# erincatto/solver2d

Hardware: NVIDIA B200
Metric: constraint_iters_per_sec (higher is better)
Workload: dtype f32

## Files before the change

### include/s2b_device.h

```cpp
#pragma once

#include <stddef.h>
#include <stdint.h>

#ifdef __cplusplus
extern "C"
{
#endif

typedef struct s2bWorld s2bWorld;

#if defined(__GNUC__)
	#define S2B_API __attribute__((visibility("default")))
#else
	#define S2B_API
#endif


#define S2B_ROW_VALID 0x1
#define S2B_BODY_ADD_FORCE 0x8

typedef struct s2bBodyRow
{
	int32_t index;
// ... 110 lines not shown
	int32_t constraintCount;
	int32_t jointCount;
	int32_t groupCount;
	int32_t overflowCount;
	int32_t treeHeight;
	int32_t movedCount;
	int32_t pairPassCount;
	int32_t kernelLaunches;
	int32_t graphReplays;
	int32_t graphCaptures;
	int64_t scratchBytes;
	int32_t regionCount;
	int32_t cutCount;
	int32_t cutGroupCount;
	int32_t recolouredCount;
} s2bCounters;


S2B_API s2bWorld* s2b_world_create(int cudaDevice, int solverType);
S2B_API void s2b_world_destroy(s2bWorld* world);

S2B_API void s2b_set_gravity(s2bWorld* world, float gx, float gy);
S2B_API void s2b_set_schedule(s2bWorld* world, int schedule);
S2B_API void s2b_set_max_colors(s2bWorld* world, int maxColors);
S2B_API void s2b_set_persistent(s2bWorld* world, int enable);
S2B_API void s2b_set_warm_gather(s2bWorld* world, int enable);
S2B_API void s2b_set_graph(s2bWorld* world, int enable);
S2B_API void s2b_set_regions(s2bWorld* world, int mode);
S2B_API void s2b_set_dataflow(s2bWorld* world, int enable);

// ... 65 lines not shown
```

### solver2d_b200/csrc/device/broadphase.cu

```cuda
#include "s2b_internal.cuh"

#include <cub/cub.cuh>
#include <thrust/iterator/counting_iterator.h>

#include <algorithm>

struct BroadScratch
{
	DevArray<int> validFlag;
	DevArray<int> leafShape;
	DevArray<unsigned> mortonIn, mortonOut;
	DevArray<int> leafIn, leafOut;
	DevArray<int> counters;
	DevArray<int> boundsBits;
	DevArray<int2> children;
	DevArray<int> parent;
	DevArray<float4> nodeBox;
	DevArray<float4> pairBox;
	DevArray<int> visit;
	DevArray<int> nodeHeight;
	DevArray<int> movedLeaves;
	DevArray<int> movedFlag;
	DevArray<int> largeShapes;
	DevArray<unsigned long long> newKey;
	DevArray<int2> newShapes;
	DevArray<int> keepFlag, keepSlots;
	DevArray<unsigned long long> mergeKeyIn, mergeKeyOut;
	DevArray<int> mergeSrcIn, mergeSrcOut;
	DevArray<char> cubTemp;
	int newPairCap = 0;
	bool treeValid = false;
	int treeShapeCap = 0;
	int treeReuses = 0;
	DevArray<unsigned long long> pairHash;
	unsigned long long hashMask = 0;
	unsigned long long hashVersion = ~0ull;
// ... 19 lines not shown
}

void s2bFreeBroadScratch(s2bWorld* w)
{
	BroadScratch* b = w->broad;
	if (b == nullptr)
	{
		return;
	}
	b->validFlag.release();
	b->leafShape.release();
	b->mortonIn.release();
	b->mortonOut.release();
	b->leafIn.release();
	b->leafOut.release();
	b->counters.release();
	b->boundsBits.release();
	b->children.release();
	b->parent.release();
	b->nodeBox.release();
	b->visit.release();
	b->nodeHeight.release();
	b->movedLeaves.release();
	b->movedFlag.release();
	b->newKey.release();
	b->newShapes.release();
	b->keepFlag.release();
	b->keepSlots.release();
	b->mergeKeyIn.release();
	b->mergeKeyOut.release();
	b->mergeSrcIn.release();
	b->mergeSrcOut.release();
	b->cubTemp.release();
	b->pairBox.release();
	b->largeShapes.release();
	b->pairHash.release();
	for (int i = 0; i < 2; ++i)
	{
		if (b->evSearch[i] != nullptr)
		{
			cudaEventDestroy(b->evSearch[i]);
		}
	}
	if (b->searchDone != nullptr)
	{
		cudaEventDestroy(b->searchDone);
	}
	delete b;
	w->broad = nullptr;
}

enum
{
	BC_LEAVES = 0,
	BC_NEW_PAIRS = 1,
	BC_KEPT = 2,
	BC_MOVED = 3,
	BC_HEIGHT = 4,
	BC_LARGE = 5,
	BC_SIZE = 8
};


__device__ __forceinline__ int s2bFloatToOrdered(float f)
{
	int i = __float_as_int(f);
	return i >= 0 ? i : i ^ 0x7FFFFFFF;
}

__device__ __forceinline__ float s2bOrderedToFloat(int i)
{
	return __int_as_float(i >= 0 ? i : i ^ 0x7FFFFFFF);
}

// ... 123 lines not shown
}

__device__ __forceinline__ int s2bPairKind(int t1, int t2)
{
	const int CAP = S2B_SHAPE_CAPSULE, CIR = S2B_SHAPE_CIRCLE, POL = S2B_SHAPE_POLYGON, SEG = S2B_SHAPE_SEGMENT;
	if (t1 == SEG && t2 == SEG)
	{
		return 0;
	}
	bool primary = (t1 == CIR && t2 == CIR) || (t1 == CAP && t2 == CIR) || (t1 == CAP && t2 == CAP) || (t1 == POL && t2 == CIR) ||
				   (t1 == POL && t2 == CAP) || (t1 == POL && t2 == POL) || (t1 == SEG && t2 != SEG);
	return primary ? 1 : 2;
}


__global__ void s2bFlagValidShapes(ShapeView s, int* validFlag)
{
	int i = blockIdx.x * blockDim.x + threadIdx.x;
	if (i < s.capacity)
	{
		validFlag[i] = (s.head[i].x & S2B_ROW_VALID) ? 1 : 0;
	}
}

__global__ void s2bSceneBounds(ShapeView s, const int* leafShape, const int* counters, int* boundsBits)
{
	int n = counters[BC_LEAVES];
	int k = blockIdx.x * blockDim.x + threadIdx.x;
	float minx = 3.0e38f, miny = 3.0e38f, maxx = -3.0e38f, maxy = -3.0e38f;
	if (k < n)
	{
		float4 f = s.fat[leafShape[k]];
		float cx = 0.5f * (f.x + f.z), cy = 0.5f * (f.y + f.w);
		minx = maxx = cx;
		miny = maxy = cy;
	}
	for (int o = 16; o > 0; o >>= 1)
	{
		minx = fminf(minx, __shfl_xor_sync(0xFFFFFFFFu, minx, o));
		miny = fminf(miny, __shfl_xor_sync(0xFFFFFFFFu, miny, o));
		maxx = fmaxf(maxx, __shfl_xor_sync(0xFFFFFFFFu, maxx, o));
		maxy = fmaxf(maxy, __shfl_xor_sync(0xFFFFFFFFu, maxy, o));
	}
	if ((threadIdx.x & 31) == 0)
	{
		atomicMin(boundsBits + 0, s2bFloatToOrdered(minx));
		atomicMin(boundsBits + 1, s2bFloatToOrdered(miny));
		atomicMax(boundsBits + 2, s2bFloatToOrdered(maxx));
		atomicMax(boundsBits + 3, s2bFloatToOrdered(maxy));
	}
}

__global__ void s2bMortonCodes(ShapeView s, const int* leafShape, const int* counters, const int* boundsBits, unsigned* morton,
							   int* leafIndex, int capacity)
{
	int n = counters[BC_LEAVES];
	int k = blockIdx.x * blockDim.x + threadIdx.x;
	if (k >= capacity)
	{
		return;
	}
	if (k >= n)
	{
		morton[k] = 0xFFFFFFFFu;
		leafIndex[k] = k;
		return;
	}
	float minx = s2bOrderedToFloat(boundsBits[0]), miny = s2bOrderedToFloat(boundsBits[1]);
	float maxx = s2bOrderedToFloat(boundsBits[2]), maxy = s2bOrderedToFloat(boundsBits[3]);
	float4 f = s.fat[leafShape[k]];
	float cx = 0.5f * (f.x + f.z), cy = 0.5f * (f.y + f.w);
	float ex = fmaxf(maxx - minx, 1.0e-6f), ey = fmaxf(maxy - miny, 1.0e-6f);
	float ux = fminf(fmaxf((cx - minx) / ex, 0.0f), 1.0f);
	float uy = fminf(fmaxf((cy - miny) / ey, 0.0f), 1.0f);
	unsigned qx = (unsigned)(ux * 32767.0f), qy = (unsigned)(uy * 32767.0f);
	morton[k] = (s2bExpandBits(qx) | (s2bExpandBits(qy) << 1)) & 0x7FFFFFFFu;
	leafIndex[k] = k;
}

__device__ __forceinline__ int s2bDelta(const unsigned* codes, int n, int i, int j)
{
	if (j < 0 || j >= n)
	{
		return -1;
	}
	unsigned a = codes[i], b = codes[j];
	if (a == b)
	{
		return 32 + __clz((unsigned)i ^ (unsigned)j);
	}
	return __clz(a ^ b);
}

__global__ void s2bBuildRadixTree(const unsigned* codes, const int* counters, int2* children, int* parent)
{
	int n = counters[BC_LEAVES];
	int i = blockIdx.x * blockDim.x + threadIdx.x;
	if (i >= n - 1)
	{
		return;
	}
	int d = (s2bDelta(codes, n, i, i + 1) - s2bDelta(codes, n, i, i - 1)) >= 0 ? 1 : -1;
	int deltaMin = s2bDelta(codes, n, i, i - d);
	int lmax = 2;
	while (s2bDelta(codes, n, i, i + lmax * d) > deltaMin)
	{
		lmax <<= 1;
	}
	int l = 0;
	for (int t = lmax >> 1; t >= 1; t >>= 1)
	{
		if (s2bDelta(codes, n, i, i + (l + t) * d) > deltaMin)
		{
			l += t;
		}
	}
	int j = i + l * d;
	int deltaNode = s2bDelta(codes, n, i, j);
	int s = 0;
	int t = l;
	do
	{
		t = (t + 1) >> 1;
		if (s2bDelta(codes, n, i, i + (s + t) * d) > deltaNode)
		{
			s += t;
		}
	} while (t > 1);
	int gamma = i + s * d + min(d, 0);
	int left = min(i, j) == gamma ? (n - 1) + gamma : gamma;
	int right = max(i, j) == gamma + 1 ? (n - 1) + gamma + 1 : gamma + 1;
	children[i] = make_int2(left, right);
	parent[left] = i;
	parent[right] = i;
	if (i == 0)
	{
		parent[0] = -1;
	}
}

__global__ void s2bRefit(ShapeView s, const int* leafShape, const int* sortedLeaf, const int* counters, const int2* children,
						 const int* parent, float4* nodeBox, float4* pairBox, int* visit, int* nodeHeight, int* countersOut)
{
	int n = counters[BC_LEAVES];
	int k = blockIdx.x * blockDim.x + threadIdx.x;
	if (k >= n)
	{
		return;
	}
	int node = (n - 1) + k;
	float4 box = s.fat[leafShape[sortedLeaf[k]]];
	nodeBox[node] = box;
	nodeHeight[node] = 0;
	if (n == 1)
	{
		countersOut[BC_HEIGHT] = 0;
		return;
	}
	int p = parent[node];
	while (p >= 0)
	{
		__threadfence();
		int arrived = atomicAdd(visit + p, 1);
		if (arrived == 0)
		{
			return;
		}
		int2 ch = children[p];
		float4 a = __ldcg(nodeBox + ch.x), b = __ldcg(nodeBox + ch.y);
		box = make_float4(fminf(a.x, b.x), fminf(a.y, b.y), fmaxf(a.z, b.z), fmaxf(a.w, b.w));
		nodeBox[p] = box;
		pairBox[2 * p] = a;
		pairBox[2 * p + 1] = b;
		int h = 1 + max(__ldcg(nodeHeight + ch.x), __ldcg(nodeHeight + ch.y));
		nodeHeight[p] = h;
		if (p == 0)
		{
			countersOut[BC_HEIGHT] = h;
		}
		p = parent[p];
	}
}


__device__ __forceinline__ void s2bBlockAppend(bool take, int value, int* list, int* count)
{
	__shared__ int warpOffset[32];
	__shared__ int blockBase;
	unsigned takers = __ballot_sync(0xFFFFFFFFu, take);
	int lane = threadIdx.x & 31, warp = threadIdx.x >> 5;
	if (lane == 0)
	{
		warpOffset[warp] = __popc(takers);
	}
	__syncthreads();
// ... 6 lines not shown
			int c = warpOffset[k];
			warpOffset[k] = total;
			total += c;
		}
		blockBase = total > 0 ? atomicAdd(count, total) : 0;
	}
	__syncthreads();
	if (take)
	{
		list[blockBase + warpOffset[warp] + __popc(takers & ((1u << lane) - 1u))] = value;
	}
}

#define S2B_MAX_LARGE_MOVERS 64

__global__ void s2bCollectMovers(ShapeView s, const int* leafShape, const int* sortedLeaf, int* counters, const float4* nodeBox, int* movedLeaves,
								 int* largeShapes)
{
	int n = counters[BC_LEAVES];
	int k = blockIdx.x * blockDim.x + threadIdx.x;
	bool moved = false;
	if (k < n)
	{
		int shape = leafShape[sortedLeaf[k]];
		moved = (s.head[shape].x & S2B_SHAPE_MOVED) != 0;
		if (moved && n >= 256)
		{
			float4 root = nodeBox[0];
			float4 box = s.fat[shape];
			float area = (box.z - box.x) * (box.w - box.y);
			float sceneArea = (root.z - root.x) * (root.w - root.y);
			if (area * 256.0f > sceneArea)
			{
				int slot = atomicAdd(counters + BC_LARGE, 1);
				if (slot < S2B_MAX_LARGE_MOVERS)
				{
					largeShapes[slot] = shape;
					moved = false;
				}
			}
		}
	}
	s2bBlockAppend(moved, k, movedLeaves, counters + BC_MOVED);
}

struct PairQuery
{
	int shapeQ, bodyQ, keyQ;
	unsigned typeBodyQ;
	int4 headQ, filterQ;
};

__device__ __forceinline__ void s2bConsiderPair(const PairQuery& q, int other, const ShapeView& s, const BodyView& b, int* counters,
												 const unsigned long long* pairHash, unsigned long long hashMask,
												 const unsigned long long* jointKeys, int jointKeyCount, unsigned long long* newKey,
												 int2* newShapes, int newCap)
{
	int shapeQ = q.shapeQ;
// ... 71 lines not shown
}

__device__ __forceinline__ bool s2bMakeQuery(PairQuery& q, int shapeQ, const ShapeView& s, const BodyView& b)
{
	q.shapeQ = shapeQ;
	q.headQ = s.head[shapeQ];
	q.filterQ = s.filter[shapeQ];
	q.bodyQ = q.headQ.y;
	q.keyQ = q.headQ.z;
	q.typeBodyQ = S2B_BODY_TYPE((unsigned)b.flags[q.bodyQ]);
	return q.typeBodyQ != S2B_BODY_STATIC;
}

#define S2B_QUERY_BATCH 16

__global__ void __launch_bounds__(128) s2bFindPairs(ShapeView s, BodyView b, const int* leafShape, const int* sortedLeaf, int* counters,
								 const int* movedLeaves, const int2* children, const float4* pairBox,
								 const unsigned long long* pairHash, unsigned long long hashMask, const unsigned long long* jointKeys,
								 int jointKeyCount, unsigned long long* newKey, int2* newShapes, int newCap)
{
	int n = counters[BC_LEAVES];
	int movedCount = counters[BC_MOVED];
	int qi = blockIdx.x * blockDim.x + threadIdx.x;
	if (qi >= movedCount)
	{
		return;
	}
	int leaf = movedLeaves[qi];
	PairQuery q;
	if (s2bMakeQuery(q, leafShape[sortedLeaf[leaf]], s, b) == false || n == 1)
	{
		return;
	}
	float4 boxQ = s.fat[q.shapeQ];

	int stack[64];
	int found[S2B_QUERY_BATCH];
	int nFound = 0;
	int sp = 0;
	int node = 0;
	bool walking = true;
	while (walking || nFound > 0)
	{
		while (walking && nFound < S2B_QUERY_BATCH)
		{
			if (node >= n - 1)
			{
				found[nFound++] = node - (n - 1);
				if (sp == 0)
				{
					walking = false;
					break;
				}
				node = stack[--sp];
				continue;
			}
			int2 ch = children[node];
			bool o0 = s2bBoxesOverlap(boxQ, pairBox[2 * node]);
			bool o1 = s2bBoxesOverlap(boxQ, pairBox[2 * node + 1]);
			if (o0 && o1)
			{
				if (sp < 64)
				{
					stack[sp++] = ch.y;
				}
				node = ch.x;
			}
			else if (o0)
			{
				node = ch.x;
			}
			else if (o1)
			{
				node = ch.y;
			}
			else
			{
				if (sp == 0)
				{
					walking = false;
					break;
				}
				node = stack[--sp];
			}
		}
		for (int k = 0; k < nFound; ++k)
		{
			s2bConsiderPair(q, leafShape[sortedLeaf[found[k]]], s, b, counters, pairHash, hashMask, jointKeys, jointKeyCount, newKey, newShapes,
							newCap);
		}
		nFound = 0;
	}
}

__global__ void s2bFindPairsLarge(ShapeView s, BodyView b, const int* leafShape, int* counters, const int* largeShapes,
								  const unsigned long long* pairHash, unsigned long long hashMask, const unsigned long long* jointKeys,
								  int jointKeyCount, unsigned long long* newKey, int2* newShapes, int newCap)
{
	int n = counters[BC_LEAVES];
	int large = min(counters[BC_LARGE], S2B_MAX_LARGE_MOVERS);
	int k = blockIdx.x * blockDim.x + threadIdx.x;
	if (k >= n || large == 0)
	{
		return;
	}
	int other = leafShape[k];
	float4 boxO = s.fat[other];
	for (int i = 0; i < large; ++i)
	{
		int shapeQ = largeShapes[i];
		if (s2bBoxesOverlap(s.fat[shapeQ], boxO) == false)
		{
			continue;
		}
		PairQuery q;
		if (s2bMakeQuery(q, shapeQ, s, b))
		{
			s2bConsiderPair(q, other, s, b, counters, pairHash, hashMask, jointKeys, jointKeyCount, newKey, newShapes, newCap);
		}
	}
}

__global__ void s2bCollectKeptContacts(ContactView c, int contactCount, ShapeView s, const unsigned long long* jointKeys, int jointKeyCount,
									   int* keepSlots, int* counters)
{
	int i = blockIdx.x * blockDim.x + threadIdx.x;
	bool keep = false;
	if (i < contactCount)
	{
		int2 sh = c.shapes[i];
		int4 ha = s.head[sh.x], hb = s.head[sh.y];
		bool alive = (ha.x & S2B_ROW_VALID) && (hb.x & S2B_ROW_VALID) && (ha.x & S2B_SHAPE_FRESH) == 0 && (hb.x & S2B_SHAPE_FRESH) == 0;
		keep = alive && s2bBoxesOverlap(s.fat[sh.x], s.fat[sh.y]) && s2bJointOverride(jointKeys, jointKeyCount, ha.y, hb.y) == false;
	}
	s2bBlockAppend(keep, i, keepSlots, counters + BC_KEPT);
}

__device__ __forceinline__ unsigned long long s2bSqueezeKey(unsigned long long pairKey, int shapeBits)
{
	return ((pairKey >> 32) << shapeBits) | (pairKey & 0xFFFFFFFFull);
}

__global__ void s2bMergeKeys(const int* counters, const int* keepSlots, const unsigned long long* oldKeys,
							 const unsigned long long* newKey, unsigned long long* mergeKey, int* mergeSrc, int capacity, int shapeBits)
{
	int kept = counters[BC_KEPT], fresh = counters[BC_NEW_PAIRS];
	int t = blockIdx.x * blockDim.x + threadIdx.x;
	if (t >= capacity)
	{
		return;
// ... 87 lines not shown

#define MAIL_BC_BASE 16

static size_t bpReserve(s2bWorld* w, BroadScratch* B)
{
	cudaStream_t st = w->stream;
	int shapeCap = w->shapeCap;
	int oldCount = w->contactCount;
	size_t nS = (size_t)shapeCap;
	B->validFlag.reserve(nS, st, false);
	B->leafShape.reserve(nS, st, false);
	B->mortonIn.reserve(nS, st, false);
	B->mortonOut.reserve(nS, st, false);
	B->leafIn.reserve(nS, st, false);
	B->leafOut.reserve(nS, st, false);
	B->counters.reserve(BC_SIZE, st, false);
	B->boundsBits.reserve(4, st, false);
	B->children.reserve(nS, st, false);
	B->parent.reserve(2 * nS, st, false);
	B->nodeBox.reserve(2 * nS, st, false);
	B->pairBox.reserve(2 * nS, st, false);
	B->visit.reserve(nS, st, false);
	B->nodeHeight.reserve(2 * nS, st, false);
	B->movedLeaves.reserve(nS, st, false);
	B->movedFlag.reserve(nS, st, false);
	B->largeShapes.reserve(S2B_MAX_LARGE_MOVERS, st, false);
	B->keepFlag.reserve((size_t)std::max(oldCount, 1), st, false);
	B->keepSlots.reserve((size_t)std::max(oldCount, 1), st, false);
	if (B->newPairCap == 0)
	{
		B->newPairCap = 8 * shapeCap + 1024;
	}
	size_t need = 0, tempBytes = 0;
	cub::DeviceSelect::Flagged(nullptr, need, thrust::counting_iterator<int>(0), (int*)nullptr, (int*)nullptr, (int*)nullptr,
							   std::max(shapeCap, oldCount), st);
	tempBytes = std::max(tempBytes, need);
	cub::DeviceRadixSort::SortPairs(nullptr, need, (unsigned*)nullptr, (unsigned*)nullptr, (int*)nullptr, (int*)nullptr, shapeCap, 0,
									32, st);
	tempBytes = std::max(tempBytes, need);
	B->newKey.reserve((size_t)B->newPairCap, st, false);
	B->newShapes.reserve((size_t)B->newPairCap, st, false);
	B->cubTemp.reserve(tempBytes + 256, st, false, false);
	return tempBytes;
}

static void bpSearch(s2bWorld* w, BroadScratch* B)
{
	cudaStream_t st = w->stream;
	int shapeCap = w->shapeCap;
	int oldCount = w->contactCount;
	ShapeView sv = shapeView(w);
	BodyView bv = bodyView(w);
	ContactColumns& cur = w->contacts[w->cur];
	size_t nS = (size_t)shapeCap;
	int newCap = B->newPairCap;

	bool reuseTree = B->treeValid && w->pairsDirty == false && B->treeShapeCap == shapeCap && B->treeReuses < S2B_TREE_REUSE_LIMIT;
	if (reuseTree)
	{
		S2B_CHECK(cudaMemsetAsync(B->counters.p + BC_NEW_PAIRS, 0, sizeof(int) * (BC_SIZE - BC_NEW_PAIRS), st));
		B->treeReuses += 1;
	}
	else
	{
		S2B_CHECK(cudaMemsetAsync(B->counters.p, 0, sizeof(int) * BC_SIZE, st));

		S2B_LAUNCH(w, s2bFlagValidShapes, gridFor(shapeCap, 256), 256, 0, sv, B->validFlag.p);
		size_t tb = B->cubTemp.cap;
		cub::DeviceSelect::Flagged(B->cubTemp.p, tb, thrust::counting_iterator<int>(0), B->validFlag.p, B->leafShape.p,
								   B->counters.p + BC_LEAVES, shapeCap, st);
		w->kernelLaunches += 2;

		int initBounds[4] = {0x7F7FFFFF, 0x7F7FFFFF, (int)0x80800000, (int)0x80800000};
		S2B_CHECK(cudaMemcpyAsync(B->boundsBits.p, initBounds, sizeof(initBounds), cudaMemcpyHostToDevice, st));
		S2B_LAUNCH(w, s2bSceneBounds, gridFor(shapeCap, 256), 256, 0, sv, B->leafShape.p, B->counters.p, B->boundsBits.p);
		S2B_LAUNCH(w, s2bMortonCodes, gridFor(shapeCap, 256), 256, 0, sv, B->leafShape.p, B->counters.p, B->boundsBits.p,
				   B->mortonIn.p, B->leafIn.p, shapeCap);
		tb = B->cubTemp.cap;
		cub::DeviceRadixSort::SortPairs(B->cubTemp.p, tb, B->mortonIn.p, B->mortonOut.p, B->leafIn.p, B->leafOut.p, shapeCap, 0, 32, st);
		w->kernelLaunches += 5;

		S2B_LAUNCH(w, s2bBuildRadixTree, gridFor(shapeCap, 256), 256, 0, B->mortonOut.p, B->counters.p, B->children.p, B->parent.p);
		B->treeValid = true;
		B->treeShapeCap = shapeCap;
		B->treeReuses = 0;
	}

	S2B_CHECK(cudaMemsetAsync(B->visit.p, 0, sizeof(int) * nS, st));
	S2B_LAUNCH(w, s2bRefit, gridFor(shapeCap, 256), 256, 0, sv, B->leafShape.p, B->leafOut.p, B->counters.p, B->children.p,
			   B->parent.p, B->nodeBox.p, B->pairBox.p, B->visit.p, B->nodeHeight.p, B->counters.p);

	if (B->hashVersion != w->contactTableVersion || B->pairHash.p == nullptr)
	{
		unsigned long long size = 1024;
		while (size < 2ull * (unsigned long long)std::max(oldCount, 1))
		{
			size <<= 1;
		}
		B->pairHash.reserve((size_t)size, st, false, false);
		B->hashMask = size - 1;
		S2B_CHECK(cudaMemsetAsync(B->pairHash.p, 0xFF, sizeof(unsigned long long) * (size_t)size, st));
		if (oldCount > 0)
		{
			S2B_LAUNCH(w, s2bBuildPairHash, gridFor(oldCount, 256), 256, 0, cur.key.p, oldCount, B->pairHash.p, B->hashMask);
		}
		B->hashVersion = w->contactTableVersion;
	}

	S2B_LAUNCH(w, s2bCollectMovers, gridFor(shapeCap, 256), 256, 0, sv, B->leafShape.p, B->leafOut.p, B->counters.p, B->nodeBox.p,
			   B->movedLeaves.p, B->largeShapes.p);
	S2B_LAUNCH(w, s2bFindPairs, gridFor(shapeCap, 128), 128, 0, sv, bv, B->leafShape.p, B->leafOut.p, B->counters.p,
			   B->movedLeaves.p, B->children.p, B->pairBox.p, B->pairHash.p, B->hashMask, w->jointPairKeys.p, w->jointPairCount,
			   B->newKey.p, B->newShapes.p, newCap);
	S2B_LAUNCH(w, s2bFindPairsLarge, gridFor(shapeCap, 256), 256, 0, sv, bv, B->leafShape.p, B->counters.p, B->largeShapes.p,
			   B->pairHash.p, B->hashMask, w->jointPairKeys.p, w->jointPairCount, B->newKey.p, B->newShapes.p, newCap);

	if (oldCount > 0)
	{
		S2B_LAUNCH(w, s2bCollectKeptContacts, gridFor(oldCount, 256), 256, 0, makeView(cur), oldCount, sv, w->jointDestroyKeys.p,
				   w->jointDestroyCount, B->keepSlots.p, B->counters.p);
	}
	S2B_CHECK(cudaMemcpyAsync(w->hostMail + MAIL_BC_BASE, B->counters.p, sizeof(int) * BC_SIZE, cudaMemcpyDeviceToHost, st));
	B->searchedCount = oldCount;
	B->searchedVersion = w->contactTableVersion;
}

static void bpCommit(s2bWorld* w, BroadScratch* B, int fresh, int kept, size_t tempBytes)
{
	cudaStream_t st = w->stream;
	int shapeCap = w->shapeCap;
	int oldCount = w->contactCount;
	ShapeView sv = shapeView(w);
	ContactColumns& cur = w->contacts[w->cur];
	ContactColumns& nxt = w->contacts[w->cur ^ 1];
	int total = kept + fresh;
	if (fresh == 0 && kept == oldCount)
// ... 95 lines not shown

	if (B->prefetched)
	{
		B->prefetched = false;
		bool valid = w->pairsDirty == false && B->prefetchEpoch == w->uploadEpoch && B->searchedVersion == w->contactTableVersion &&
					 B->searchedCount == w->contactCount && w->prefetchPairs == 1;
		if (valid)
		{
			S2B_CHECK(cudaEventSynchronize(B->searchDone));
			S2B_CHECK(cudaEventRecord(w->timer.ev[0], st));
			const int* hc = w->hostMail + MAIL_BC_BASE;
			int fresh = hc[BC_NEW_PAIRS], kept = hc[BC_KEPT];
			if (fresh <= B->newPairCap)
			{
				w->treeHeight = hc[BC_HEIGHT];
				B->lastPassRan = hc[BC_MOVED] > 0 || hc[BC_LARGE] > 0;
				bpCommit(w, B, fresh, kept, B->prefetchTempBytes);
				return;
			}
			B->newPairCap = fresh + fresh / 2 + 1024;
		}
	}

	bool run = w->pairsDirty;
	if (run == false)
	{
		if (w->movedEvent != nullptr)
		{
			S2B_CHECK(cudaEventSynchronize(w->movedEvent));
		}
// ... 11 lines not shown
	}

	for (int attempt = 0; attempt < 4; ++attempt)
	{
		size_t tempBytes = bpReserve(w, B);
		bpSearch(w, B);
		S2B_CHECK(cudaStreamSynchronize(st));
		const int* hc = w->hostMail + MAIL_BC_BASE;
		int fresh = hc[BC_NEW_PAIRS], kept = hc[BC_KEPT];
		if (fresh > B->newPairCap)
		{
			B->newPairCap = fresh + fresh / 2 + 1024;
			continue;
		}
		w->treeHeight = hc[BC_HEIGHT];
		bpCommit(w, B, fresh, kept, tempBytes);
		break;
	}
}
```

### solver2d_b200/csrc/device/s2b_internal.cuh

```cuda
#pragma once

#include "s2b_device.h"
#include "solver2d/constants.h"
#include "solver2d/aabb.h"
#include "solver2d/math.h"

#include <cuda_runtime.h>
#include <stdint.h>
#include <stdio.h>
#include <stdlib.h>
#include <string.h>
#include <vector>

#define S2B_CHECK(call)                                                                                                \
	do                                                                                                                 \
	{                                                                                                                  \
		cudaError_t err__ = (call);                                                                                    \
		if (err__ != cudaSuccess)                                                                                      \
		{                                                                                                              \
			fprintf(stderr, "solver2d-b200: CUDA error %s at %s:%d (%s) — no CPU fallback, aborting\n",                 \
					cudaGetErrorString(err__), __FILE__, __LINE__, #call);                                             \
			abort();                                                                                                   \
		}                                                                                                              \
	} while (0)
// ... 298 lines not shown
	int contactCount = 0;
	bool sticky = false;

	bool pairsDirty = true;
	unsigned long long uploadEpoch = 0;
	int prefetchPairs = 1;
	int kempe = 1;
	int wholeIslandBodies = 1200;
	int residentRegions = 1;
	int hubDegree = 48;
	int fusePositions = 1;
	int kempeGrid = 0;
	DevArray<int> dMovedFlag;
	int pairPassCount = 0;
	int treeHeight = 0;

	std::vector<unsigned long long> orderHint;

	struct SolverScratch* scratch = nullptr;
	struct BroadScratch* broad = nullptr;

	int* hostMail = nullptr;
	int* devMail = nullptr;

	int kernelLaunches = 0;
	DevArray<unsigned long long> dWork;
	cudaEvent_t solveKernelStart = nullptr, solveKernelEnd = nullptr;
	bool solveKernelTimed = false;
	cudaEvent_t markEvents[2] = {nullptr, nullptr};
	cudaEvent_t movedEvent = nullptr;
// ... 90 lines not shown
```

### solver2d_b200/csrc/device/solver.cu

```cuda
#include "persistent.cuh"

#include <cooperative_groups.h>
#include <cuda/barrier>
#include <cub/cub.cuh>
#include <thrust/iterator/counting_iterator.h>

#include <algorithm>

namespace cg = cooperative_groups;


SolverScratch* s2bGetSolverScratch(s2bWorld* w)
{
	if (w->scratch == nullptr)
	{
		w->scratch = new SolverScratch();
	}
	return w->scratch;
}

void s2bFreeSolverScratch(s2bWorld* w)
{
	SolverScratch* s = w->scratch;
	if (s == nullptr)
// ... 3340 lines not shown
			S2B_CHECK(cudaMemcpy(ks, w->scratch->kempeState.p, sizeof(ks), cudaMemcpyDeviceToHost));
			out->recolouredCount = ks[KS_FIXED];
		}
		if (w->scratch->bodyTicket.p != nullptr && w->scratch->flowErrorOffset > 0)
		{
			int flag = 0;
			S2B_CHECK(cudaMemcpy(&flag, w->scratch->bodyTicket.p + w->scratch->flowErrorOffset, sizeof(int), cudaMemcpyDeviceToHost));
			if (flag != 0)
			{
				fprintf(stderr, "solver2d-b200: a ticketed solver pass ran into its spin limit (internal error)\n");
				abort();
			}
		}
	}
	out->treeHeight = w->treeHeight;
	out->movedCount = w->hostMail[MAIL_MOVED];
	out->pairPassCount = w->pairPassCount;
	out->kernelLaunches = w->kernelLaunches;
	out->graphReplays = w->scratch != nullptr ? w->scratch->graphReplays : 0;
	out->graphCaptures = w->scratch != nullptr ? w->scratch->graphCaptures : 0;
}

extern "C" void s2b_set_solve_trace(s2bWorld* w, int capacity)
{
	s2bGetSolverScratch(w)->traceCap = capacity > 0 ? capacity + 1 : 0;
}

extern "C" int s2b_get_solve_trace(s2bWorld* w, uint64_t* out, int maxEntries)
{
	S2B_CHECK(cudaSetDevice(w->device));
// ... 86 lines not shown
```

### solver2d_b200/device.py

```python
from __future__ import annotations

import ctypes as C
import os

import numpy as np

HERE = os.path.dirname(os.path.abspath(__file__))
LIB_PATH = os.path.join(HERE, "libsolver2d.so")

BODY_ROW = np.dtype([
    ("index", "<i4"), ("flags", "<i4"), ("origin", "<f4", 2), ("position", "<f4", 2), ("rot", "<f4", 2),
    ("linearVelocity", "<f4", 2), ("angularVelocity", "<f4"), ("localCenter", "<f4", 2), ("mass", "<f4"),
    ("invMass", "<f4"), ("I", "<f4"), ("invI", "<f4"), ("force", "<f4", 2), ("torque", "<f4"),
    ("linearDamping", "<f4"), ("angularDamping", "<f4"), ("gravityScale", "<f4"),
], align=True)

SHAPE_ROW = np.dtype([
    ("index", "<i4"), ("flags", "<i4"), ("body", "<i4"), ("proxyKey", "<i4"), ("categoryBits", "<u4"),
    ("maskBits", "<u4"), ("groupIndex", "<i4"), ("friction", "<f4"), ("aabb", "<f4", 4), ("fatAABB", "<f4", 4),
    ("radius", "<f4"), ("count", "<i4"), ("vertices", "<f4", 16), ("normals", "<f4", 16),
], align=True)

JOINT_ROW = np.dtype([
    ("index", "<i4"), ("flags", "<i4"), ("bodyA", "<i4"), ("bodyB", "<i4"), ("localOriginAnchorA", "<f4", 2),
# ... 14 lines not shown
    ("cacheCount", "<i4"), ("cacheIndexA", "u1", 4), ("cacheIndexB", "u1", 4), ("cacheMetric", "<f4"),
], align=True)


class StepContext(C.Structure):
    _fields_ = [("dt", C.c_float), ("inv_dt", C.c_float), ("h", C.c_float), ("inv_h", C.c_float),
                ("iterations", C.c_int32), ("extraIterations", C.c_int32), ("warmStart", C.c_int32)]


class Counters(C.Structure):
    _fields_ = [("bodyCapacity", C.c_int32), ("shapeCapacity", C.c_int32), ("jointCapacity", C.c_int32),
                ("contactCount", C.c_int32), ("constraintCount", C.c_int32), ("jointCount", C.c_int32),
                ("groupCount", C.c_int32), ("overflowCount", C.c_int32), ("treeHeight", C.c_int32),
                ("movedCount", C.c_int32), ("pairPassCount", C.c_int32), ("kernelLaunches", C.c_int32),
                ("graphReplays", C.c_int32), ("graphCaptures", C.c_int32), ("scratchBytes", C.c_int64),
                ("regionCount", C.c_int32), ("cutCount", C.c_int32), ("cutGroupCount", C.c_int32), ("recolouredCount", C.c_int32)]


SCHEDULE_COLOR, SCHEDULE_WAVEFRONT = 0, 1
ROW_VALID = 0x1
SHAPE_MOVED = 0x10
JOINT_ENABLE_LIMIT, JOINT_ENABLE_MOTOR, JOINT_COLLIDE_CONNECTED = 0x10, 0x20, 0x40

ABI_SYMBOLS = [
    "s2b_world_create", "s2b_world_destroy", "s2b_set_gravity", "s2b_set_schedule", "s2b_set_max_colors",
    "s2b_set_persistent", "s2b_upload_bodies", "s2b_upload_shapes", "s2b_upload_joints", "s2b_upload_contacts",
    "s2b_upload_joint_pairs", "s2b_mark_pairs_dirty", "s2b_set_contact_order", "s2b_update_pairs",
    "s2b_update_contacts", "s2b_solve", "s2b_finalize", "s2b_step", "s2b_sync", "s2b_download_bodies",
    "s2b_download_all_bodies", "s2b_download_shape_boxes", "s2b_download_joints", "s2b_download_contacts",
    "s2b_download_solve_order", "s2b_download_islands", "s2b_prefetch_pairs", "s2b_get_counters", "s2b_pack_body_state", "s2b_timed_steps", "s2b_last_stage_ms",
    "s2b_flush_l2", "s2b_time_color_kernel", "s2b_version", "s2b_abi_sizes", "s2b_upload_forces", "s2b_host_alloc",
# ... 223 lines not shown
```

Before: 5.526 billion.

## Replace binary radix BVH with flat 16-ary Morton-sorted hierarchy in broadphase

```diff
diff --git a/include/s2b_device.h b/include/s2b_device.h
--- a/include/s2b_device.h
+++ b/include/s2b_device.h
@@ -148,6 +148,8 @@
 	int32_t cutCount;
 	int32_t cutGroupCount;
 	int32_t recolouredCount;
+	int32_t largeLeafCount;
+	int32_t pairRebuildCount;
 } s2bCounters;
 
 
diff --git a/solver2d_b200/csrc/device/broadphase.cu b/solver2d_b200/csrc/device/broadphase.cu
--- a/solver2d_b200/csrc/device/broadphase.cu
+++ b/solver2d_b200/csrc/device/broadphase.cu
@@ -11,15 +11,11 @@
 	DevArray<int> leafShape;
 	DevArray<unsigned> mortonIn, mortonOut;
 	DevArray<int> leafIn, leafOut;
+	DevArray<int> sortedShape;
 	DevArray<int> counters;
 	DevArray<int> boundsBits;
-	DevArray<int2> children;
-	DevArray<int> parent;
 	DevArray<float4> nodeBox;
-	DevArray<float4> pairBox;
-	DevArray<int> visit;
-	DevArray<int> nodeHeight;
-	DevArray<int> movedLeaves;
+	DevArray<int> movedShapes;
 	DevArray<int> movedFlag;
 	DevArray<int> largeShapes;
 	DevArray<unsigned long long> newKey;
@@ -69,14 +65,11 @@
 	b->mortonOut.release();
 	b->leafIn.release();
 	b->leafOut.release();
+	b->sortedShape.release();
 	b->counters.release();
 	b->boundsBits.release();
-	b->children.release();
-	b->parent.release();
 	b->nodeBox.release();
-	b->visit.release();
-	b->nodeHeight.release();
-	b->movedLeaves.release();
+	b->movedShapes.release();
 	b->movedFlag.release();
 	b->newKey.release();
 	b->newShapes.release();
@@ -87,7 +80,6 @@
 	b->mergeSrcIn.release();
 	b->mergeSrcOut.release();
 	b->cubTemp.release();
-	b->pairBox.release();
 	b->largeShapes.release();
 	b->pairHash.release();
 	for (int i = 0; i < 2; ++i)
@@ -108,11 +100,13 @@
 enum
 {
 	BC_LEAVES = 0,
-	BC_NEW_PAIRS = 1,
-	BC_KEPT = 2,
-	BC_MOVED = 3,
-	BC_HEIGHT = 4,
-	BC_LARGE = 5,
+	BC_LARGE_LEAVES = 1,
+	BC_NEW_PAIRS = 2,
+	BC_KEPT = 3,
+	BC_MOVED = 4,
+	BC_HEIGHT = 5,
+	BC_LARGE = 6,
+	BC_REFIT_DONE = 7,
 	BC_SIZE = 8
 };
 
@@ -266,6 +260,49 @@
 }
 
 
+#define S2B_FANOUT 16
+#define S2B_MAX_LEVELS 8
+
+#define S2B_MAX_LARGE_LEAVES 64
+
+__device__ __forceinline__ int s2bLevels(int n, int nh, int* offset, int* count)
+{
+	offset[0] = 0;
+	count[0] = nh;
+	int top = 0, off = n;
+	while (count[top] > S2B_FANOUT && top + 1 < S2B_MAX_LEVELS)
+	{
+		int c = (count[top] + S2B_FANOUT - 1) / S2B_FANOUT;
+		top += 1;
+		offset[top] = off;
+		count[top] = c;
+		off += c;
+	}
+	return top;
+}
+
+__device__ __forceinline__ float4 s2bEmptyBox()
+{
+	return make_float4(3.0e38f, 3.0e38f, -3.0e38f, -3.0e38f);
+}
+
+__device__ __forceinline__ float4 s2bUnion(float4 a, float4 b)
+{
+	return make_float4(fminf(a.x, b.x), fminf(a.y, b.y), fmaxf(a.z, b.z), fmaxf(a.w, b.w));
+}
+
+__device__ __forceinline__ float4 s2bUnion16(float4 box)
+{
+	for (int o = S2B_FANOUT / 2; o > 0; o >>= 1)
+	{
+		box.x = fminf(box.x, __shfl_xor_sync(0xFFFFFFFFu, box.x, o));
+		box.y = fminf(box.y, __shfl_xor_sync(0xFFFFFFFFu, box.y, o));
+		box.z = fmaxf(box.z, __shfl_xor_sync(0xFFFFFFFFu, box.z, o));
+		box.w = fmaxf(box.w, __shfl_xor_sync(0xFFFFFFFFu, box.w, o));
+	}
+	return box;
+}
+
 __global__ void s2bFlagValidShapes(ShapeView s, int* validFlag)
 {
 	int i = blockIdx.x * blockDim.x + threadIdx.x;
@@ -279,31 +316,41 @@
 {
 	int n = counters[BC_LEAVES];
 	int k = blockIdx.x * blockDim.x + threadIdx.x;
-	float minx = 3.0e38f, miny = 3.0e38f, maxx = -3.0e38f, maxy = -3.0e38f;
+	float c[4] = {3.0e38f, 3.0e38f, -3.0e38f, -3.0e38f};
+	float4 box = s2bEmptyBox();
 	if (k < n)
 	{
-		float4 f = s.fat[leafShape[k]];
-		float cx = 0.5f * (f.x + f.z), cy = 0.5f * (f.y + f.w);
-		minx = maxx = cx;
-		miny = maxy = cy;
-	}
+		box = s.fat[leafShape[k]];
+		float cx = 0.5f * (box.x + box.z), cy = 0.5f * (box.y + box.w);
+		c[0] = c[2] = cx;
+		c[1] = c[3] = cy;
+	}
+	float v[8] = {c[0], c[1], c[2], c[3], box.x, box.y, box.z, box.w};
 	for (int o = 16; o > 0; o >>= 1)
 	{
-		minx = fminf(minx, __shfl_xor_sync(0xFFFFFFFFu, minx, o));
-		miny = fminf(miny, __shfl_xor_sync(0xFFFFFFFFu, miny, o));
-		maxx = fmaxf(maxx, __shfl_xor_sync(0xFFFFFFFFu, maxx, o));
-		maxy = fmaxf(maxy, __shfl_xor_sync(0xFFFFFFFFu, maxy, o));
+		for (int j = 0; j < 8; ++j)
+		{
+			float u = __shfl_xor_sync(0xFFFFFFFFu, v[j], o);
+			v[j] = (j & 2) ? fmaxf(v[j], u) : fminf(v[j], u);
+		}
 	}
 	if ((threadIdx.x & 31) == 0)
 	{
-		atomicMin(boundsBits + 0, s2bFloatToOrdered(minx));
-		atomicMin(boundsBits + 1, s2bFloatToOrdered(miny));
-		atomicMax(boundsBits + 2, s2bFloatToOrdered(maxx));
-		atomicMax(boundsBits + 3, s2bFloatToOrdered(maxy));
-	}
-}
-
-__global__ void s2bMortonCodes(ShapeView s, const int* leafShape, const int* counters, const int* boundsBits, unsigned* morton,
+		for (int j = 0; j < 8; ++j)
+		{
+			if (j & 2)
+			{
+				atomicMax(boundsBits + j, s2bFloatToOrdered(v[j]));
+			}
+			else
+			{
+				atomicMin(boundsBits + j, s2bFloatToOrdered(v[j]));
+			}
+		}
+	}
+}
+
+__global__ void s2bMortonCodes(ShapeView s, const int* leafShape, int* counters, const int* boundsBits, unsigned* morton,
 							   int* leafIndex, int capacity)
 {
 	int n = counters[BC_LEAVES];
@@ -312,125 +359,40 @@
 	{
 		return;
 	}
+	leafIndex[k] = k;
 	if (k >= n)
 	{
 		morton[k] = 0xFFFFFFFFu;
-		leafIndex[k] = k;
 		return;
 	}
 	float minx = s2bOrderedToFloat(boundsBits[0]), miny = s2bOrderedToFloat(boundsBits[1]);
 	float maxx = s2bOrderedToFloat(boundsBits[2]), maxy = s2bOrderedToFloat(boundsBits[3]);
 	float4 f = s.fat[leafShape[k]];
+	if (n >= 256)
+	{
+		float sceneSide = fmaxf(s2bOrderedToFloat(boundsBits[6]) - s2bOrderedToFloat(boundsBits[4]),
+								s2bOrderedToFloat(boundsBits[7]) - s2bOrderedToFloat(boundsBits[5]));
+		float side = fmaxf(f.z - f.x, f.w - f.y);
+		if (side * 16.0f > sceneSide && atomicAdd(counters + BC_LARGE_LEAVES, 1) < S2B_MAX_LARGE_LEAVES)
+		{
+			morton[k] = 0xFFFFFFFFu;
+			return;
+		}
+	}
 	float cx = 0.5f * (f.x + f.z), cy = 0.5f * (f.y + f.w);
 	float ex = fmaxf(maxx - minx, 1.0e-6f), ey = fmaxf(maxy - miny, 1.0e-6f);
 	float ux = fminf(fmaxf((cx - minx) / ex, 0.0f), 1.0f);
 	float uy = fminf(fmaxf((cy - miny) / ey, 0.0f), 1.0f);
 	unsigned qx = (unsigned)(ux * 32767.0f), qy = (unsigned)(uy * 32767.0f);
 	morton[k] = (s2bExpandBits(qx) | (s2bExpandBits(qy) << 1)) & 0x7FFFFFFFu;
-	leafIndex[k] = k;
-}
-
-__device__ __forceinline__ int s2bDelta(const unsigned* codes, int n, int i, int j)
-{
-	if (j < 0 || j >= n)
-	{
-		return -1;
-	}
-	unsigned a = codes[i], b = codes[j];
-	if (a == b)
-	{
-		return 32 + __clz((unsigned)i ^ (unsigned)j);
-	}
-	return __clz(a ^ b);
-}
-
-__global__ void s2bBuildRadixTree(const unsigned* codes, const int* counters, int2* children, int* parent)
-{
-	int n = counters[BC_LEAVES];
-	int i = blockIdx.x * blockDim.x + threadIdx.x;
-	if (i >= n - 1)
-	{
-		return;
-	}
-	int d = (s2bDelta(codes, n, i, i + 1) - s2bDelta(codes, n, i, i - 1)) >= 0 ? 1 : -1;
-	int deltaMin = s2bDelta(codes, n, i, i - d);
-	int lmax = 2;
-	while (s2bDelta(codes, n, i, i + lmax * d) > deltaMin)
-	{
-		lmax <<= 1;
-	}
-	int l = 0;
-	for (int t = lmax >> 1; t >= 1; t >>= 1)
-	{
-		if (s2bDelta(codes, n, i, i + (l + t) * d) > deltaMin)
-		{
-			l += t;
-		}
-	}
-	int j = i + l * d;
-	int deltaNode = s2bDelta(codes, n, i, j);
-	int s = 0;
-	int t = l;
-	do
-	{
-		t = (t + 1) >> 1;
-		if (s2bDelta(codes, n, i, i + (s + t) * d) > deltaNode)
-		{
-			s += t;
-		}
-	} while (t > 1);
-	int gamma = i + s * d + min(d, 0);
-	int left = min(i, j) == gamma ? (n - 1) + gamma : gamma;
-	int right = max(i, j) == gamma + 1 ? (n - 1) + gamma + 1 : gamma + 1;
-	children[i] = make_int2(left, right);
-	parent[left] = i;
-	parent[right] = i;
-	if (i == 0)
-	{
-		parent[0] = -1;
-	}
-}
-
-__global__ void s2bRefit(ShapeView s, const int* leafShape, const int* sortedLeaf, const int* counters, const int2* children,
-						 const int* parent, float4* nodeBox, float4* pairBox, int* visit, int* nodeHeight, int* countersOut)
-{
-	int n = counters[BC_LEAVES];
+}
+
+__global__ void s2bSortedShapes(const int* leafShape, const int* leafOut, const int* counters, int* sortedShape)
+{
 	int k = blockIdx.x * blockDim.x + threadIdx.x;
-	if (k >= n)
-	{
-		return;
-	}
-	int node = (n - 1) + k;
-	float4 box = s.fat[leafShape[sortedLeaf[k]]];
-	nodeBox[node] = box;
-	nodeHeight[node] = 0;
-	if (n == 1)
-	{
-		countersOut[BC_HEIGHT] = 0;
-		return;
-	}
-	int p = parent[node];
-	while (p >= 0)
-	{
-		__threadfence();
-		int arrived = atomicAdd(visit + p, 1);
-		if (arrived == 0)
-		{
-			return;
-		}
-		int2 ch = children[p];
-		float4 a = __ldcg(nodeBox + ch.x), b = __ldcg(nodeBox + ch.y);
-		box = make_float4(fminf(a.x, b.x), fminf(a.y, b.y), fmaxf(a.z, b.z), fmaxf(a.w, b.w));
-		nodeBox[p] = box;
-		pairBox[2 * p] = a;
-		pairBox[2 * p + 1] = b;
-		int h = 1 + max(__ldcg(nodeHeight + ch.x), __ldcg(nodeHeight + ch.y));
-		nodeHeight[p] = h;
-		if (p == 0)
-		{
-			countersOut[BC_HEIGHT] = h;
-		}
-		p = parent[p];
+	if (k < counters[BC_LEAVES])
+	{
+		sortedShape[k] = leafShape[leafOut[k]];
 	}
 }
 
@@ -467,22 +429,26 @@
 
 #define S2B_MAX_LARGE_MOVERS 64
 
-__global__ void s2bCollectMovers(ShapeView s, const int* leafShape, const int* sortedLeaf, int* counters, const float4* nodeBox, int* movedLeaves,
-								 int* largeShapes)
+__global__ void __launch_bounds__(256) s2bRefit(ShapeView s, const int* sortedShape, int* counters, const int* boundsBits,
+												 float4* nodeBox, int* movedShapes, int* largeShapes)
 {
 	int n = counters[BC_LEAVES];
+	int nh = n - min(counters[BC_LARGE_LEAVES], S2B_MAX_LARGE_LEAVES);
 	int k = blockIdx.x * blockDim.x + threadIdx.x;
 	bool moved = false;
+	int shape = -1;
+	float4 box = s2bEmptyBox();
 	if (k < n)
 	{
-		int shape = leafShape[sortedLeaf[k]];
+		shape = sortedShape[k];
+		box = s.fat[shape];
+		nodeBox[k] = box;
 		moved = (s.head[shape].x & S2B_SHAPE_MOVED) != 0;
 		if (moved && n >= 256)
 		{
-			float4 root = nodeBox[0];
-			float4 box = s.fat[shape];
+			float sceneArea = (s2bOrderedToFloat(boundsBits[6]) - s2bOrderedToFloat(boundsBits[4])) *
+							  (s2bOrderedToFloat(boundsBits[7]) - s2bOrderedToFloat(boundsBits[5]));
 			float area = (box.z - box.x) * (box.w - box.y);
-			float sceneArea = (root.z - root.x) * (root.w - root.y);
 			if (area * 256.0f > sceneArea)
 			{
 				int slot = atomicAdd(counters + BC_LARGE, 1);
@@ -494,7 +460,60 @@
 			}
 		}
 	}
-	s2bBlockAppend(moved, k, movedLeaves, counters + BC_MOVED);
+	s2bBlockAppend(moved, shape, movedShapes, counters + BC_MOVED);
+
+	int offset[S2B_MAX_LEVELS], count[S2B_MAX_LEVELS];
+	int top = s2bLevels(n, nh, offset, count);
+	__shared__ float4 level1[256 / S2B_FANOUT];
+	__shared__ bool lastBlock;
+	float4 group = s2bUnion16(k < nh ? box : s2bEmptyBox());
+	if ((threadIdx.x & (S2B_FANOUT - 1)) == 0)
+	{
+		if (top >= 1 && k < nh)
+		{
+			nodeBox[offset[1] + k / S2B_FANOUT] = group;
+		}
+		level1[threadIdx.x / S2B_FANOUT] = group;
+	}
+	__syncthreads();
+	if (threadIdx.x < 32)
+	{
+		float4 node = s2bUnion16(threadIdx.x < 256 / S2B_FANOUT ? level1[threadIdx.x] : s2bEmptyBox());
+		if (threadIdx.x == 0 && top >= 2 && blockIdx.x * 256 < nh)
+		{
+			nodeBox[offset[2] + blockIdx.x] = node;
+		}
+	}
+	if (threadIdx.x == 0)
+	{
+		__threadfence();
+		lastBlock = atomicAdd(counters + BC_REFIT_DONE, 1) == (int)gridDim.x - 1;
+	}
+	__syncthreads();
+	if (lastBlock == false)
+	{
+		return;
+	}
+	__threadfence();
+	for (int l = 3; l <= top; ++l)
+	{
+		const float4* below = nodeBox + offset[l - 1];
+		for (int i = threadIdx.x; i < count[l]; i += blockDim.x)
+		{
+			int first = i * S2B_FANOUT, last = min(first + S2B_FANOUT, count[l - 1]);
+			float4 r = s2bEmptyBox();
+			for (int j = first; j < last; ++j)
+			{
+				r = s2bUnion(r, __ldcg(below + j));
+			}
+			nodeBox[offset[l] + i] = r;
+		}
+		__syncthreads();
+	}
+	if (threadIdx.x == 0)
+	{
+		counters[BC_HEIGHT] = top + 1;
+	}
 }
 
 struct PairQuery
@@ -596,82 +615,110 @@
 
 #define S2B_QUERY_BATCH 16
 
-__global__ void __launch_bounds__(128) s2bFindPairs(ShapeView s, BodyView b, const int* leafShape, const int* sortedLeaf, int* counters,
-								 const int* movedLeaves, const int2* children, const float4* pairBox,
-								 const unsigned long long* pairHash, unsigned long long hashMask, const unsigned long long* jointKeys,
-								 int jointKeyCount, unsigned long long* newKey, int2* newShapes, int newCap)
-{
+__device__ __forceinline__ unsigned s2bOverlapMask(const float4* __restrict__ boxes, int count, float4 q)
+{
+	unsigned mask = 0;
+#pragma unroll
+	for (int j = 0; j < S2B_FANOUT; ++j)
+	{
+		if (j < count && s2bBoxesOverlap(q, __ldg(boxes + j)))
+		{
+			mask |= 1u << j;
+		}
+	}
+	return mask;
+}
+
+__device__ __forceinline__ void s2bCollectKeptContacts(int i, const ContactView& c, int contactCount, const ShapeView& s,
+														const unsigned long long* jointKeys, int jointKeyCount, int* keepSlots, int* counters)
+{
+	bool keep = false;
+	if (i < contactCount)
+	{
+		int2 sh = c.shapes[i];
+		int4 ha = s.head[sh.x], hb = s.head[sh.y];
+		bool alive = (ha.x & S2B_ROW_VALID) && (hb.x & S2B_ROW_VALID) && (ha.x & S2B_SHAPE_FRESH) == 0 && (hb.x & S2B_SHAPE_FRESH) == 0;
+		keep = alive && s2bBoxesOverlap(s.fat[sh.x], s.fat[sh.y]) && s2bJointOverride(jointKeys, jointKeyCount, ha.y, hb.y) == false;
+	}
+	s2bBlockAppend(keep, i, keepSlots, counters + BC_KEPT);
+}
+
+__global__ void __launch_bounds__(128) s2bFindPairs(ShapeView s, BodyView b, const int* sortedShape, int* counters, const int* movedShapes,
+													const float4* __restrict__ nodeBox, int queryBlocks, ContactView cur, int contactCount,
+													const unsigned long long* destroyKeys, int destroyKeyCount, int* keepSlots,
+													const unsigned long long* pairHash, unsigned long long hashMask,
+													const unsigned long long* jointKeys, int jointKeyCount, unsigned long long* newKey,
+													int2* newShapes, int newCap)
+{
+	if ((int)blockIdx.x >= queryBlocks)
+	{
+		s2bCollectKeptContacts(((int)blockIdx.x - queryBlocks) * blockDim.x + threadIdx.x, cur, contactCount, s, destroyKeys,
+							   destroyKeyCount, keepSlots, counters);
+		return;
+	}
 	int n = counters[BC_LEAVES];
+	int large = min(counters[BC_LARGE_LEAVES], S2B_MAX_LARGE_LEAVES);
+	int nh = n - large;
 	int movedCount = counters[BC_MOVED];
 	int qi = blockIdx.x * blockDim.x + threadIdx.x;
 	if (qi >= movedCount)
 	{
 		return;
 	}
-	int leaf = movedLeaves[qi];
 	PairQuery q;
-	if (s2bMakeQuery(q, leafShape[sortedLeaf[leaf]], s, b) == false || n == 1)
+	if (s2bMakeQuery(q, movedShapes[qi], s, b) == false)
 	{
 		return;
 	}
 	float4 boxQ = s.fat[q.shapeQ];
 
-	int stack[64];
-	int found[S2B_QUERY_BATCH];
+	int offset[S2B_MAX_LEVELS], count[S2B_MAX_LEVELS];
+	int top = s2bLevels(n, nh, offset, count);
+	unsigned pending[S2B_MAX_LEVELS];
+	int base[S2B_MAX_LEVELS];
+	int found[S2B_QUERY_BATCH + S2B_FANOUT];
 	int nFound = 0;
-	int sp = 0;
-	int node = 0;
-	bool walking = true;
+	int level = top;
+	bool walking = nh > 0;
+	if (walking)
+	{
+		pending[top] = s2bOverlapMask(nodeBox + offset[top], count[top], boxQ);
+		base[top] = 0;
+	}
 	while (walking || nFound > 0)
 	{
 		while (walking && nFound < S2B_QUERY_BATCH)
 		{
-			if (node >= n - 1)
+			unsigned m = pending[level];
+			if (level == 0 || m == 0)
 			{
-				found[nFound++] = node - (n - 1);
-				if (sp == 0)
+				for (; m != 0; m &= m - 1)
 				{
-					walking = false;
-					break;
+					found[nFound++] = base[0] + __ffs(m) - 1;
 				}
-				node = stack[--sp];
+				level += 1;
+				walking = level <= top;
 				continue;
 			}
-			int2 ch = children[node];
-			bool o0 = s2bBoxesOverlap(boxQ, pairBox[2 * node]);
-			bool o1 = s2bBoxesOverlap(boxQ, pairBox[2 * node + 1]);
-			if (o0 && o1)
-			{
-				if (sp < 64)
-				{
-					stack[sp++] = ch.y;
-				}
-				node = ch.x;
-			}
-			else if (o0)
-			{
-				node = ch.x;
-			}
-			else if (o1)
-			{
-				node = ch.y;
-			}
-			else
-			{
-				if (sp == 0)
-				{
-					walking = false;
-					break;
-				}
-				node = stack[--sp];
-			}
+			pending[level] = m & (m - 1);
+			int first = (base[level] + __ffs(m) - 1) * S2B_FANOUT;
+			pending[level - 1] = s2bOverlapMask(nodeBox + offset[level - 1] + first, min(S2B_FANOUT, count[level - 1] - first), boxQ);
+			base[level - 1] = first;
+			level -= 1;
 		}
 		for (int k = 0; k < nFound; ++k)
 		{
-			s2bConsiderPair(q, leafShape[sortedLeaf[found[k]]], s, b, counters, pairHash, hashMask, jointKeys, jointKeyCount, newKey, newShapes,
+			s2bConsiderPair(q, sortedShape[found[k]], s, b, counters, pairHash, hashMask, jointKeys, jointKeyCount, newKey, newShapes,
 							newCap);
 		}
 		nFound = 0;
+	}
+	for (int i = nh; i < n; ++i)
+	{
+		if (s2bBoxesOverlap(boxQ, nodeBox[i]))
+		{
+			s2bConsiderPair(q, sortedShape[i], s, b, counters, pairHash, hashMask, jointKeys, jointKeyCount, newKey, newShapes, newCap);
+		}
 	}
 }
 
@@ -701,21 +748,6 @@
 			s2bConsiderPair(q, other, s, b, counters, pairHash, hashMask, jointKeys, jointKeyCount, newKey, newShapes, newCap);
 		}
 	}
-}
-
-__global__ void s2bCollectKeptContacts(ContactView c, int contactCount, ShapeView s, const unsigned long long* jointKeys, int jointKeyCount,
-									   int* keepSlots, int* counters)
-{
-	int i = blockIdx.x * blockDim.x + threadIdx.x;
-	bool keep = false;
-	if (i < contactCount)
-	{
-		int2 sh = c.shapes[i];
-		int4 ha = s.head[sh.x], hb = s.head[sh.y];
-		bool alive = (ha.x & S2B_ROW_VALID) && (hb.x & S2B_ROW_VALID) && (ha.x & S2B_SHAPE_FRESH) == 0 && (hb.x & S2B_SHAPE_FRESH) == 0;
-		keep = alive && s2bBoxesOverlap(s.fat[sh.x], s.fat[sh.y]) && s2bJointOverride(jointKeys, jointKeyCount, ha.y, hb.y) == false;
-	}
-	s2bBlockAppend(keep, i, keepSlots, counters + BC_KEPT);
 }
 
 __device__ __forceinline__ unsigned long long s2bSqueezeKey(unsigned long long pairKey, int shapeBits)
@@ -833,15 +865,11 @@
 	B->mortonOut.reserve(nS, st, false);
 	B->leafIn.reserve(nS, st, false);
 	B->leafOut.reserve(nS, st, false);
+	B->sortedShape.reserve(nS, st, false);
 	B->counters.reserve(BC_SIZE, st, false);
-	B->boundsBits.reserve(4, st, false);
-	B->children.reserve(nS, st, false);
-	B->parent.reserve(2 * nS, st, false);
-	B->nodeBox.reserve(2 * nS, st, false);
-	B->pairBox.reserve(2 * nS, st, false);
-	B->visit.reserve(nS, st, false);
-	B->nodeHeight.reserve(2 * nS, st, false);
-	B->movedLeaves.reserve(nS, st, false);
+	B->boundsBits.reserve(8, st, false);
+	B->nodeBox.reserve(nS + nS / 8 + 64, st, false);
+	B->movedShapes.reserve(nS, st, false);
 	B->movedFlag.reserve(nS, st, false);
 	B->largeShapes.reserve(S2B_MAX_LARGE_MOVERS, st, false);
 	B->keepFlag.reserve((size_t)std::max(oldCount, 1), st, false);
@@ -871,7 +899,6 @@
 	ShapeView sv = shapeView(w);
 	BodyView bv = bodyView(w);
 	ContactColumns& cur = w->contacts[w->cur];
-	size_t nS = (size_t)shapeCap;
 	int newCap = B->newPairCap;
 
 	bool reuseTree = B->treeValid && w->pairsDirty == false && B->treeShapeCap == shapeCap && B->treeReuses < S2B_TREE_REUSE_LIMIT;
@@ -890,7 +917,8 @@
 								   B->counters.p + BC_LEAVES, shapeCap, st);
 		w->kernelLaunches += 2;
 
-		int initBounds[4] = {0x7F7FFFFF, 0x7F7FFFFF, (int)0x80800000, (int)0x80800000};
+		const int lo = 0x7F7FFFFF, hi = (int)0x80800000;
+		int initBounds[8] = {lo, lo, hi, hi, lo, lo, hi, hi};
 		S2B_CHECK(cudaMemcpyAsync(B->boundsBits.p, initBounds, sizeof(initBounds), cudaMemcpyHostToDevice, st));
 		S2B_LAUNCH(w, s2bSceneBounds, gridFor(shapeCap, 256), 256, 0, sv, B->leafShape.p, B->counters.p, B->boundsBits.p);
 		S2B_LAUNCH(w, s2bMortonCodes, gridFor(shapeCap, 256), 256, 0, sv, B->leafShape.p, B->counters.p, B->boundsBits.p,
@@ -898,16 +926,15 @@
 		tb = B->cubTemp.cap;
 		cub::DeviceRadixSort::SortPairs(B->cubTemp.p, tb, B->mortonIn.p, B->mortonOut.p, B->leafIn.p, B->leafOut.p, shapeCap, 0, 32, st);
 		w->kernelLaunches += 5;
-
-		S2B_LAUNCH(w, s2bBuildRadixTree, gridFor(shapeCap, 256), 256, 0, B->mortonOut.p, B->counters.p, B->children.p, B->parent.p);
+		S2B_LAUNCH(w, s2bSortedShapes, gridFor(shapeCap, 256), 256, 0, B->leafShape.p, B->leafOut.p, B->counters.p, B->sortedShape.p);
 		B->treeValid = true;
 		B->treeShapeCap = shapeCap;
 		B->treeReuses = 0;
-	}
-
-	S2B_CHECK(cudaMemsetAsync(B->visit.p, 0, sizeof(int) * nS, st));
-	S2B_LAUNCH(w, s2bRefit, gridFor(shapeCap, 256), 256, 0, sv, B->leafShape.p, B->leafOut.p, B->counters.p, B->children.p,
-			   B->parent.p, B->nodeBox.p, B->pairBox.p, B->visit.p, B->nodeHeight.p, B->counters.p);
+		w->pairRebuildCount += 1;
+	}
+
+	S2B_LAUNCH(w, s2bRefit, gridFor(shapeCap, 256), 256, 0, sv, B->sortedShape.p, B->counters.p, B->boundsBits.p, B->nodeBox.p,
+			   B->movedShapes.p, B->largeShapes.p);
 
 	if (B->hashVersion != w->contactTableVersion || B->pairHash.p == nullptr)
 	{
@@ -926,19 +953,13 @@
 		B->hashVersion = w->contactTableVersion;
 	}
 
-	S2B_LAUNCH(w, s2bCollectMovers, gridFor(shapeCap, 256), 256, 0, sv, B->leafShape.p, B->leafOut.p, B->counters.p, B->nodeBox.p,
-			   B->movedLeaves.p, B->largeShapes.p);
-	S2B_LAUNCH(w, s2bFindPairs, gridFor(shapeCap, 128), 128, 0, sv, bv, B->leafShape.p, B->leafOut.p, B->counters.p,
-			   B->movedLeaves.p, B->children.p, B->pairBox.p, B->pairHash.p, B->hashMask, w->jointPairKeys.p, w->jointPairCount,
-			   B->newKey.p, B->newShapes.p, newCap);
+	int queryBlocks = gridFor(shapeCap, 128);
+	S2B_LAUNCH(w, s2bFindPairs, queryBlocks + (oldCount > 0 ? gridFor(oldCount, 128) : 0), 128, 0, sv, bv, B->sortedShape.p,
+			   B->counters.p, B->movedShapes.p, B->nodeBox.p, queryBlocks, makeView(cur), oldCount, w->jointDestroyKeys.p,
+			   w->jointDestroyCount, B->keepSlots.p, B->pairHash.p, B->hashMask, w->jointPairKeys.p, w->jointPairCount, B->newKey.p,
+			   B->newShapes.p, newCap);
 	S2B_LAUNCH(w, s2bFindPairsLarge, gridFor(shapeCap, 256), 256, 0, sv, bv, B->leafShape.p, B->counters.p, B->largeShapes.p,
 			   B->pairHash.p, B->hashMask, w->jointPairKeys.p, w->jointPairCount, B->newKey.p, B->newShapes.p, newCap);
-
-	if (oldCount > 0)
-	{
-		S2B_LAUNCH(w, s2bCollectKeptContacts, gridFor(oldCount, 256), 256, 0, makeView(cur), oldCount, sv, w->jointDestroyKeys.p,
-				   w->jointDestroyCount, B->keepSlots.p, B->counters.p);
-	}
 	S2B_CHECK(cudaMemcpyAsync(w->hostMail + MAIL_BC_BASE, B->counters.p, sizeof(int) * BC_SIZE, cudaMemcpyDeviceToHost, st));
 	B->searchedCount = oldCount;
 	B->searchedVersion = w->contactTableVersion;
@@ -1064,6 +1085,7 @@
 			if (fresh <= B->newPairCap)
 			{
 				w->treeHeight = hc[BC_HEIGHT];
+				w->largeLeafCount = std::min(hc[BC_LARGE_LEAVES], S2B_MAX_LARGE_LEAVES);
 				B->lastPassRan = hc[BC_MOVED] > 0 || hc[BC_LARGE] > 0;
 				bpCommit(w, B, fresh, kept, B->prefetchTempBytes);
 				return;
@@ -1105,6 +1127,7 @@
 			continue;
 		}
 		w->treeHeight = hc[BC_HEIGHT];
+		w->largeLeafCount = std::min(hc[BC_LARGE_LEAVES], S2B_MAX_LARGE_LEAVES);
 		bpCommit(w, B, fresh, kept, tempBytes);
 		break;
 	}
diff --git a/solver2d_b200/csrc/device/s2b_internal.cuh b/solver2d_b200/csrc/device/s2b_internal.cuh
--- a/solver2d_b200/csrc/device/s2b_internal.cuh
+++ b/solver2d_b200/csrc/device/s2b_internal.cuh
@@ -336,6 +336,8 @@
 	DevArray<int> dMovedFlag;
 	int pairPassCount = 0;
 	int treeHeight = 0;
+	int largeLeafCount = 0;
+	int pairRebuildCount = 0;
 
 	std::vector<unsigned long long> orderHint;
 
diff --git a/solver2d_b200/csrc/device/solver.cu b/solver2d_b200/csrc/device/solver.cu
--- a/solver2d_b200/csrc/device/solver.cu
+++ b/solver2d_b200/csrc/device/solver.cu
@@ -3378,6 +3378,8 @@
 		}
 	}
 	out->treeHeight = w->treeHeight;
+	out->largeLeafCount = w->largeLeafCount;
+	out->pairRebuildCount = w->pairRebuildCount;
 	out->movedCount = w->hostMail[MAIL_MOVED];
 	out->pairPassCount = w->pairPassCount;
 	out->kernelLaunches = w->kernelLaunches;
diff --git a/solver2d_b200/device.py b/solver2d_b200/device.py
--- a/solver2d_b200/device.py
+++ b/solver2d_b200/device.py
@@ -52,7 +52,8 @@
                 ("groupCount", C.c_int32), ("overflowCount", C.c_int32), ("treeHeight", C.c_int32),
                 ("movedCount", C.c_int32), ("pairPassCount", C.c_int32), ("kernelLaunches", C.c_int32),
                 ("graphReplays", C.c_int32), ("graphCaptures", C.c_int32), ("scratchBytes", C.c_int64),
-                ("regionCount", C.c_int32), ("cutCount", C.c_int32), ("cutGroupCount", C.c_int32), ("recolouredCount", C.c_int32)]
+                ("regionCount", C.c_int32), ("cutCount", C.c_int32), ("cutGroupCount", C.c_int32), ("recolouredCount", C.c_int32),
+                ("largeLeafCount", C.c_int32), ("pairRebuildCount", C.c_int32)]
 
 
 SCHEDULE_COLOR, SCHEDULE_WAVEFRONT = 0, 1
```

Result: faster. 5.883 billion (median of 6 runs) (+6.5%).
